# SciML/NeuralPDE.jl

Measured on NVIDIA H100. Metric: collocation-points/sec (loss+grad), higher is better.
Workload: dtype f32

## Files before the change

### neuralpde.jl_b200/csrc/tc_common.cuh

```cuda
#pragma once
#include <cuda_runtime.h>
#include <stdint.h>
#include "tc_types.h"
#include "ffma_kernel.cuh"
#include "tc_prims.cuh"
#include "tail.cuh"

namespace pinn {

constexpr int kNH = kTcThreads / 128;
static_assert(kTcThreads == 512, "the MMA chains are spread over four warpgroups");
constexpr int GW = 4;
constexpr int GWB = 2;

template <int N>
__device__ __forceinline__ float pick(const float* v, int idx) {
  float r = v[0];
#pragma unroll
  for (int i = 1; i < N; ++i) r = (idx == i) ? v[i] : r;
  return r;
}
template <int N>
__device__ __forceinline__ void add_at(float* v, int idx, float x) {
#pragma unroll
// ... 194 lines not shown
  int tl_max, off_P, off_misc, off_ones, mx_dim, mx_taps;
};
__device__ __forceinline__ void cta_base_init(CtaBase& cs, const TcCommonArgs& a, float* partial) {
  cs.partial = partial;
  cs.tl_max = a.tl_max; cs.off_P = a.off_P; cs.off_misc = a.off_misc; cs.off_ones = a.off_ones;
  cs.mx_dim = a.mx_dim; cs.mx_taps = a.mx_taps;
#ifdef PINN_DEBUG
  cs.dbg = (blockIdx.x == 0) ? a.dbg : nullptr;
#else
  cs.dbg = nullptr;
#endif
  cs.dbg_n = 0;
  dbg_mark(&cs, 1);
}

struct Misc {
  float *Xs, *taps, *tapbar, *scratch, *qws;
  double* tsum;
  uint64_t* bar_ld;
};
__device__ __forceinline__ Misc misc_of(uint8_t* m, int mx_dim, int mx_taps) {
  Misc r;
  r.Xs = reinterpret_cast<float*>(m);             m += mx_dim * kTcPts * 4;
  r.taps = reinterpret_cast<float*>(m);           m += mx_taps * kTcPts * 4;
  r.tapbar = reinterpret_cast<float*>(m);         m += mx_taps * kTcPts * 4;
  r.scratch = reinterpret_cast<float*>(m);        m += kTcMaxC * kTcPts * 4;
  r.qws = reinterpret_cast<float*>(m);            m += kTcPts * 4;
  r.tsum = reinterpret_cast<double*>(m);          m += PINN_MAX_TERMS * 8;
  r.bar_ld = reinterpret_cast<uint64_t*>(m);
  return r;
}

template <int N1, int N2>
struct PassInfo {
  int L, TL, d_in, n1w, nL;
  int dir1[N1 > 0 ? N1 : 1];
  Chan<N1, N2> ch;
};
template <int N1, int N2>
__device__ __forceinline__ void load_pass(PassInfo<N1, N2>& pi, const DevNet& net, const DevChan& dc) {
  pi.L = net.n_layers; pi.TL = pi.L - 2; pi.d_in = net.dims[0]; pi.n1w = net.dims[1]; pi.nL = net.dims[pi.L - 1];
#pragma unroll
  for (int j = 0; j < N1; ++j) pi.dir1[j] = dc.dir1[j];
#pragma unroll
  for (int s = 0; s < N2; ++s) { pi.ch.sa[s] = dc.s_a[s]; pi.ch.sb[s] = dc.s_b[s]; }
}

template <int W, int N1, int N2>
__device__ __forceinline__ void first_layer_elem(uint32_t fpa, const PassInfo<N1, N2>& pi, const float (&x)[PINN_MAX_IN],
                                                 int o, float* zz) {
  using F = FpBlock<W>;
  float s = lds_f32(fpa + (F::B1 + o) * 4);
  const uint32_t wa = fpa + (F::W1 + o * 8) * 4;
  if (pi.d_in <= 3) {
    s = fmaf(lds_f32(wa), x[0], s);
    if (pi.d_in >= 2) s = fmaf(lds_f32(wa + 4), x[1], s);
    if (pi.d_in == 3) s = fmaf(lds_f32(wa + 8), x[2], s);
  } else {
#pragma unroll
    for (int k = 0; k < PINN_MAX_IN; ++k)
      if (k < pi.d_in) s = fmaf(lds_f32(wa + k * 4), x[k], s);
  }
  zz[0] = s;
#pragma unroll
  for (int j = 0; j < N1; ++j) zz[1 + j] = lds_f32(fpa + (F::W1 + o * 8 + pi.dir1[j]) * 4);
#pragma unroll
  for (int j = 0; j < N2; ++j) zz[1 + N1 + j] = 0.f;
}

__device__ __forceinline__ void wait_bar(uint64_t* bar, uint32_t& phase) {
  tc::mbar_wait(bar, phase);
  phase ^= 1u;
}

static __device__ __noinline__ void mma_chain(uint32_t d, uint64_t adesc, uint64_t bdesc, uint32_t a_step, uint32_t b_step, int nk,
                                          uint32_t idesc, uint32_t acc_first) {
  const int n = (int)(idesc & 0xffu), ta = (int)((idesc >> 8) & 1u), tb = (int)((idesc >> 9) & 1u);
  const uint32_t dcol = d & 0xffffu, j = dcol >> 4;
  const uint32_t lbo = (uint32_t)((adesc >> 16) & 0x3fffu) << 4;
  const int wg = (int)(threadIdx.x >> 7);
#pragma unroll 1
  for (int h = 0; h < 2; ++h) {
    if (h == 1 && ta && lbo == 0) break;
    if (wg != 2 * (__popc(j) & 1) + h) continue;
    const uint64_t a = adesc + ((h ? (ta ? lbo : 8192u) : 0u) >> 4);
    if (ta == 0 && tb == 0) tc::wg_chain_n<0, 0>(n, dcol, h, a, bdesc, a_step, b_step, nk, acc_first);
    else if (ta == 0) tc::wg_chain_n<0, 1>(n, dcol, h, a, bdesc, a_step, b_step, nk, acc_first);
    else if (tb == 0) tc::wg_chain_n<1, 0>(n, dcol, h, a, bdesc, a_step, b_step, nk, acc_first);
    else tc::wg_chain_n<1, 1>(n, dcol, h, a, bdesc, a_step, b_step, nk, acc_first);
  }
}

struct Tid {
  int tid, warp, lane, q, hh, p;
  uint32_t lane_addr;
};
__device__ __forceinline__ Tid tid_of() {
  Tid t;
  t.tid = threadIdx.x; t.warp = t.tid >> 5; t.lane = t.tid & 31; t.q = t.warp & 3; t.hh = t.warp >> 2;
  t.p = t.q * 32 + t.lane;
  t.lane_addr = (uint32_t)(t.q * 32) << 16;
  return t;
}


__device__ __forceinline__ void cta_setup(const TcCommonArgs& a, const Misc& ms, float* partial, long long n_theta, bool want_grad) {
  extern __shared__ __align__(1024) uint8_t smem[];
  const int tid = threadIdx.x;
  if (want_grad) {
    const long long n4 = n_theta / 4;
    float4* p4 = reinterpret_cast<float4*>(partial);
    if ((reinterpret_cast<uintptr_t>(partial) & 15) == 0) {
      for (long long i = tid; i < n4; i += kTcThreads) p4[i] = make_float4(0.f, 0.f, 0.f, 0.f);
      for (long long i = n4 * 4 + tid; i < n_theta; i += kTcThreads) partial[i] = 0.f;
    } else {
      for (long long i = tid; i < n_theta; i += kTcThreads) partial[i] = 0.f;
    }
  }
  if (tid < PINN_MAX_TERMS) ms.tsum[tid] = 0.0;
  if (tid < 64) {
    const int r = tid >> 3, ch = tid & 7;
    *reinterpret_cast<uint4*>(smem + a.off_ones + r * 128 + ch * 16) = make_uint4(ch == r ? 0x00003f80u : 0u, 0u, 0u, 0u);
  }
}

template <int W>
__device__ __forceinline__ void stage_fp_block(float* fp, const DevNet& net, const float* theta) {
  using F = FpBlock<W>;
  const int tid = threadIdx.x, L = net.n_layers;
  for (int i = tid; i < F::SIZE; i += kTcThreads) fp[i] = 0.f;
  __syncthreads();
  const int n1w = net.dims[1], d_in = net.dims[0];
  const long long w0 = net.w_off[0], b0 = net.b_off[0];
  for (int i = tid; i < n1w * d_in; i += kTcThreads) {
    const int o = i % n1w, k = i / n1w;
    fp[F::W1 + o * 8 + k] = __ldg(&theta[w0 + i]);
  }
  for (int i = tid; i < n1w; i += kTcThreads) fp[F::B1 + i] = __ldg(&theta[b0 + i]);
  for (int i = tid; i < (L - 2) * W; i += kTcThreads) {
    const int l = 1 + i / W, o = i & (W - 1);
    if (o < net.dims[l + 1]) fp[F::BT + (l - 1) * W + o] = __ldg(&theta[net.b_off[l] + o]);
  }
  const int nL = net.dims[L - 1];
  const long long wl = net.w_off[L - 1], bl = net.b_off[L - 1];
  for (int i = tid; i < nL; i += kTcThreads) fp[F::WL + i] = __ldg(&theta[wl + i]);
  if (tid == 0) fp[F::BL] = __ldg(&theta[bl]);
}

struct TileRef {
  int ti;
  long long p0, n_pts;
};

__device__ __forceinline__ TileRef stage_tile(const TcCommonArgs& a, const DevProblem& P, const Misc& ms, int tile,
                                              uint32_t& ld_phase) {
  const int tid = threadIdx.x;
  int ti = 0;
  while (ti + 1 < P.n_terms && tile >= a.dyn[ti + 1].tile0) ++ti;
  const DevTerm& tm = P.terms[ti];
  const long long p0 = (long long)(tile - a.dyn[ti].tile0) * kTcPts;
  const long long n_pts = a.dyn[ti].n;
  const float* pts = reinterpret_cast<const float*>(a.dyn[ti].pts);
  const float* qw = reinterpret_cast<const float*>(a.dyn[ti].qw);
  if (tid < (int)((sizeof(DevTerm) + 127) / 128)) tc::prefetch_l1(reinterpret_cast<const char*>(&tm) + tid * 128);
  const int dim = tm.dim, n_taps = tm.n_taps, weighted = tm.weighted;
  const float* tile_src = pts + p0 * dim;
  const bool bulk_tile = (p0 + kTcPts <= n_pts) && dim <= kTcMaxC && ((reinterpret_cast<uintptr_t>(tile_src) & 15) == 0);
  if (bulk_tile) {
    if (tid == 0) {
      tc::mbar_arrive_expect_tx(ms.bar_ld, (uint32_t)(dim * kTcPts * 4));
      tc::bulk_load(ms.scratch, tile_src, (uint32_t)(dim * kTcPts * 4), ms.bar_ld);
    }
    wait_bar(ms.bar_ld, ld_phase);
    if (tid < kTcPts)
      for (int r = 0; r < dim; ++r) ms.Xs[r * kTcPts + tid] = ms.scratch[tid * dim + r];
  } else {
    for (int i = tid; i < dim * kTcPts; i += kTcThreads) {
      int pp = i / dim, r = i - pp * dim;
      long long gp = p0 + pp;
      if (gp >= n_pts) gp = n_pts - 1;
      ms.Xs[r * kTcPts + pp] = pts[gp * dim + r];
    }
  }
  if (tid < kTcPts) {
    long long gp = p0 + tid;
    float w = 0.f;
    if (gp < n_pts) w = weighted ? qw[gp] : 1.f;
    ms.qws[tid] = w;
  }
  for (int i = tid; i < n_taps * kTcPts; i += kTcThreads) ms.tapbar[i] = 0.f;
  __syncthreads();
  return TileRef{ti, p0, n_pts};
}

__device__ __forceinline__ void residual_step(const TcCommonArgs& a, const DevProblem& P, const DevTerm& tm, const Misc& ms,
                                              const TileRef& tr, uint8_t* region, size_t region_bytes, float* partial,
                                              bool want_grad) {
  const int tid = threadIdx.x, lane = tid & 31;
  const int n_instr = tm.n_instr, n_taps = tm.n_taps;
  DevInstr* sprog = reinterpret_cast<DevInstr*>(region);
  float* sval = reinterpret_cast<float*>(region + 8192);
  const bool prog_sm = (size_t)8192 + (size_t)2 * n_instr * kTcPts * 4 <= region_bytes;
  if (prog_sm) {
    const int nw = n_instr * (int)(sizeof(DevInstr) / 4);
    const int* src = reinterpret_cast<const int*>(tm.prog);
    for (int i = tid; i < nw; i += kTcThreads) reinterpret_cast<int*>(sprog)[i] = __ldg(src + i);
    __syncthreads();
  }
  if (tid < kTcPts) {
    float pbar[PINN_MAX_PARAMS];
#pragma unroll
    for (int j = 0; j < PINN_MAX_PARAMS; ++j) pbar[j] = 0.f;
    float r;
    if (prog_sm) {
      r = run_program_t<float, kTcPts, true>(sprog, n_instr, a.theta + P.param_off, ms.Xs, ms.taps, ms.tapbar, pbar, tid,
                                             want_grad, sval, sval + n_instr * kTcPts);
    } else {
      r = run_program<float, kTcPts>(tm, a.theta + P.param_off, ms.Xs, ms.taps, ms.tapbar, pbar, tid, want_grad);
    }
    const float w = ms.qws[tid];
    double s = (double)w * (double)r * (double)r;
#pragma unroll
    for (int o = 16; o > 0; o >>= 1) s += __shfl_xor_sync(0xffffffffu, s, o);
    if (lane == 0) atomicAdd(&ms.tsum[tr.ti], s);
    if (a.mode == 2) {
      long long gp = tr.p0 + tid;
      if (gp < tr.n_pts) a.resid_out[gp] = r;
    }
    if (want_grad) {
      const float g = (float)a.seed[tr.ti] * w * 2.f * r;
      for (int tt = 0; tt < n_taps; ++tt) ms.tapbar[tt * kTcPts + tid] *= g;
      const int n_params = P.n_params;
      for (int j = 0; j < n_params; ++j) {
        float v = warp_sum<float>(pbar[j] * g);
        if (lane == 0) atomicAdd(&partial[P.param_off + j], v);
      }
    }
  }
  __syncthreads();
}

struct DbgSpan {
  long long c0;
  unsigned long long g0;
};
__device__ __forceinline__ DbgSpan dbg_span_begin(const long long* dbg) {
  DbgSpan s{0, 0};
#ifdef PINN_DEBUG
  if (dbg && threadIdx.x == 0) {
    s.c0 = clock64();
    asm volatile("mov.u64 %0, %globaltimer;" : "=l"(s.g0));
  }
#endif
  return s;
}

template <typename CS>
__device__ __forceinline__ void cta_finish(const TcCommonArgs& a, const CS& cs, const DbgSpan& span, const Misc& ms,
                                           const DevProblem& P, bool want_grad) {
  extern __shared__ __align__(1024) uint8_t smem[];
  const int tid = threadIdx.x;
#ifdef PINN_DEBUG
  if (tid == 0 && cs.dbg) cs.dbg[999] = cs.dbg_n;
  if (a.dbg && tid == 0 && blockIdx.x < 250) {
    unsigned long long g1;
    unsigned int smid;
    asm volatile("mov.u64 %0, %globaltimer;" : "=l"(g1));
    asm volatile("mov.u32 %0, %smid;" : "=r"(smid));
    long long* rec = a.dbg + 1000 + 4 * blockIdx.x;
    rec[0] = (long long)span.g0; rec[1] = (long long)g1; rec[2] = clock64() - span.c0; rec[3] = smid;
  }
#endif
  if (tid < PINN_MAX_TERMS) a.term_sums[(long long)blockIdx.x * PINN_MAX_TERMS + tid] = ms.tsum[tid];
  if (a.tail.state)
    fused_tail<float, kTcThreads>(a.tail, a.partial, a.partial_stride, a.term_sums, P.n_theta, P.n_terms, want_grad ? 1 : 0,
                                  reinterpret_cast<float*>(smem + a.off_P));
}


template <int C, typename CS>
__device__ __forceinline__ void finish_forward(CS* cs, const DevTerm& tm, int slot, const Misc& ms, const float* bl, const Tid& t,
                                               const float (&u)[C]) {
  __syncthreads();
  dbg_mark(cs, 15);
#pragma unroll
  for (int c = 0; c < C; ++c) atomicAdd(&ms.scratch[c * kTcPts + t.p], u[c]);
  __syncthreads();
  if (t.hh == 0) {
    float s[C];
#pragma unroll
    for (int c = 0; c < C; ++c) s[c] = ms.scratch[c * kTcPts + t.p];
    s[0] += *bl;
    const int n_taps = tm.n_taps;
    for (int tt = 0; tt < n_taps; ++tt)
      if (tm.tap_slot[tt] == slot) {
        const int tch = tm.tap_ch[tt];
        float v = s[0];
#pragma unroll
        for (int c = 1; c < C; ++c) v = (tch == c) ? s[c] : v;
        ms.taps[tt * kTcPts + t.p] = v;
      }
  }
  __syncthreads();
  dbg_mark(cs, 16);
}

template <int C>
__device__ __forceinline__ void gather_ubar(const DevTerm& tm, int slot, const Misc& ms, int p, float (&ub)[C]) {
#pragma unroll
  for (int c = 0; c < C; ++c) ub[c] = 0.f;
  const int n_taps = tm.n_taps;
  for (int tt = 0; tt < n_taps; ++tt)
    if (tm.tap_slot[tt] == slot) {
      const float g = ms.tapbar[tt * kTcPts + p];
      const int tch = tm.tap_ch[tt];
#pragma unroll
      for (int c = 0; c < C; ++c) ub[c] += (tch == c) ? g : 0.f;
    }
}

template <int C>
__device__ __forceinline__ void last_layer_grad(const Tid& t, const float (&ub)[C], int nL, float* gw, float* gb, uint32_t u_tile,
// ... 149 lines not shown
```

### neuralpde.jl_b200/csrc/tc_kernel.cu

```cuda
#include "tc_common.cuh"

namespace pinn {

using Fp = FpBlock<kTcW>;

struct CtaShared : CtaBase {
  int split, off_Q;
  uint8_t* stash;
  TcNetSmem nets[PINN_MAX_NETS];
};

struct LoopCtx {
  uint32_t fp;
  uint32_t bt;
  uint32_t tP;
  uint32_t tQ;
  float* gb;
  float* gw;
  uint32_t taddr;
  int act, split, p, lane, g0, g1, flag;
  __device__ __forceinline__ LoopCtx(uint32_t fp_, uint32_t bt_, uint32_t tP_, uint32_t tQ_, const Tid& t, int act_, int ng,
                                     int flag_, int split_ = 0, float* gb_ = nullptr, float* gw_ = nullptr)
      : fp(fp_), bt(bt_), tP(tP_), tQ(tQ_), gb(gb_), gw(gw_), taddr(t.lane_addr), act(act_), split(split_), p(t.p), lane(t.lane),
        g0(t.hh * (ng / kNH)), g1((t.hh + 1) * (ng / kNH)), flag(flag_) {}
// ... 20 lines not shown
      for (int c = 0; c < C; ++c) zz[c] = mk2(za[c], zb2[c]);
      chain_fwd<N1, N2, PURE, AK, P2>(lc.act, pi.ch, zz, hv);
#pragma unroll
      for (int c = 0; c < C; ++c) { h[c][i] = hv[c].v.x; h[c][i + 1] = hv[c].v.y; }
      if (lc.flag) {
        const float w0 = lds_f32(lc.fp + (Fp::WL + g * GW + i) * 4), w1 = lds_f32(lc.fp + (Fp::WL + g * GW + i + 1) * 4);
#pragma unroll
        for (int c = 0; c < C; ++c) u[c] = fmaf(w1, hv[c].v.y, fmaf(w0, hv[c].v.x, u[c]));
      }
    }
#pragma unroll
    for (int c = 0; c < C; ++c) store_half(lc.tP + c * kTileBytes, lc.tQ + c * kTileBytes, lc.p, g * GW, h[c], lc.split != 0);
  }
#pragma unroll
  for (int c = 0; c < C; ++c) up[c] = u[c];
}

template <int C, int NK, bool SPLIT>
__device__ __forceinline__ void fwd_mma(float (&d)[C][16], uint32_t sP, uint32_t sQ, uint32_t whi, uint32_t wlo) {
  const int wg = threadIdx.x >> 7;
  const uint32_t aoff = (wg & 1) * 8192u, boff = (wg >> 1) * 32u * 128u;
  const uint64_t dwhi = tc::make_desc(whi + boff, 0, 1024), dwlo = tc::make_desc(wlo + boff, 0, 1024);
  tc::wgmma_fence();
#pragma unroll
  for (int c = 0; c < C; ++c) {
    const uint64_t dahi = tc::make_desc(sP + c * kTileBytes + aoff, 0, 1024);
    const uint64_t dalo = tc::make_desc(sQ + c * kTileBytes + aoff, 0, 1024);
#pragma unroll
    for (int pr = 0; pr < (SPLIT ? 3 : 1); ++pr) {
      const uint64_t a = (pr == 2) ? dalo : dahi, b = (pr == 1) ? dwlo : dwhi;
#pragma unroll
      for (int k = 0; k < NK; ++k)
        tc::wgmma_n32<0, 0>(d[c], a + 2 * k, b + 2 * k, (pr | k) ? 1u : 0u);
    }
  }
  tc::wgmma_commit();
  tc::wgmma_wait0();
}
template <int C>
__device__ __forceinline__ void fwd_mma_any(float (&d)[C][16], uint32_t sP, uint32_t sQ, uint32_t whi, uint32_t wlo, int nk,
                                            bool split) {
  switch (nk * 2 + (split ? 1 : 0)) {
    case 2: fwd_mma<C, 1, false>(d, sP, sQ, whi, wlo); break;
    case 3: fwd_mma<C, 1, true>(d, sP, sQ, whi, wlo); break;
    case 4: fwd_mma<C, 2, false>(d, sP, sQ, whi, wlo); break;
    case 5: fwd_mma<C, 2, true>(d, sP, sQ, whi, wlo); break;
    case 6: fwd_mma<C, 3, false>(d, sP, sQ, whi, wlo); break;
    case 7: fwd_mma<C, 3, true>(d, sP, sQ, whi, wlo); break;
    case 8: fwd_mma<C, 4, false>(d, sP, sQ, whi, wlo); break;
    default: fwd_mma<C, 4, true>(d, sP, sQ, whi, wlo); break;
  }
}

template <int N1, int N2, bool PURE, int AK, int C>
__device__ __forceinline__ void tl_fwd_frag(const float (&d)[C][16], const LoopCtx lc, const Chan<N1, N2> ch, float* scratch) {
  const int wg = threadIdx.x >> 7, w = (threadIdx.x >> 5) & 3;
  const int row0 = 64 * (wg & 1) + 16 * w + (lc.lane >> 2);
  const int col0 = 32 * (wg >> 1) + 2 * (lc.lane & 3);
  float u[2][C];
#pragma unroll
  for (int r = 0; r < 2; ++r)
#pragma unroll
    for (int c = 0; c < C; ++c) u[r][c] = 0.f;
#pragma unroll
  for (int i = 0; i < 16; i += 2) {
    const int rh = (i >> 1) & 1;
    const int row = row0 + 8 * rh, col = col0 + 8 * (i >> 2);
    P2 zz[C], hv[C];
    zz[0] = mk2(d[0][i] + lds_f32(lc.bt + col * 4), d[0][i + 1] + lds_f32(lc.bt + (col + 1) * 4));
#pragma unroll
    for (int c = 1; c < C; ++c) zz[c] = mk2(d[c][i], d[c][i + 1]);
    chain_fwd<N1, N2, PURE, AK, P2>(lc.act, ch, zz, hv);
    const uint32_t off = tc::swz_off(row, col);
#pragma unroll
    for (int c = 0; c < C; ++c) {
      const uint32_t hx = tc::pack_bf16(hv[c].v.x, hv[c].v.y);
      asm volatile("st.shared.b32 [%0], %1;" ::"r"(lc.tP + c * kTileBytes + off), "r"(hx) : "memory");
      if (lc.split)
        asm volatile("st.shared.b32 [%0], %1;" ::"r"(lc.tQ + c * kTileBytes + off), "r"(bf16x2_lo(hv[c].v.x, hv[c].v.y, hx))
                     : "memory");
    }
    if (lc.flag) {
      const float w0 = lds_f32(lc.fp + (Fp::WL + col) * 4), w1 = lds_f32(lc.fp + (Fp::WL + col + 1) * 4);
#pragma unroll
      for (int c = 0; c < C; ++c) u[rh][c] = fmaf(w1, hv[c].v.y, fmaf(w0, hv[c].v.x, u[rh][c]));
    }
  }
  if (lc.flag) {
#pragma unroll
    for (int r = 0; r < 2; ++r)
#pragma unroll
      for (int c = 0; c < C; ++c) {
        float s = u[r][c];
        s += __shfl_xor_sync(0xffffffffu, s, 1);
        s += __shfl_xor_sync(0xffffffffu, s, 2);
        if ((lc.lane & 3) == 0) atomicAdd(&scratch[c * kTcPts + row0 + 8 * r], s);
      }
  }
}

template <int C, int NKO>
__device__ __forceinline__ void dgrad_mma(float (&d)[C][16], uint32_t sP, uint32_t whi) {
  const uint32_t poff = (threadIdx.x >> 7) * 32u * 128u;
  const uint64_t dw = tc::make_desc(whi, 0, 1024);
  tc::wgmma_fence();
#pragma unroll
  for (int c = 0; c < C; ++c) {
    const uint64_t dz = tc::make_desc(sP + c * kTileBytes + poff, 0, 1024);
#pragma unroll
    for (int k = 0; k < NKO; ++k)
      tc::wgmma_n32<1, 0>(d[c], dw + 128 * k, dz + 2 * k, k ? 1u : 0u);
  }
  tc::wgmma_commit();
  tc::wgmma_wait0();
}
template <int C>
__device__ __forceinline__ void dgrad_mma_any(float (&d)[C][16], uint32_t sP, uint32_t whi, int nko) {
  switch (nko) {
    case 1: dgrad_mma<C, 1>(d, sP, whi); break;
    case 2: dgrad_mma<C, 2>(d, sP, whi); break;
    case 3: dgrad_mma<C, 3>(d, sP, whi); break;
    default: dgrad_mma<C, 4>(d, sP, whi); break;
  }
}
template <int C>
__device__ __forceinline__ void wgrad_mma(float (&dw)[32], float (&db)[8], uint32_t sP, uint32_t sQ, uint32_t s_ones) {
  const uint32_t poff = (threadIdx.x >> 7) * 32u * 128u;
  const uint64_t d1 = tc::make_desc(s_ones, 0, 0);
  tc::wgmma_fence();
#pragma unroll
  for (int c = 0; c < C; ++c) {
    const uint64_t dh = tc::make_desc(sQ + c * kTileBytes + poff, 0, 1024), dz = tc::make_desc(sP + c * kTileBytes + poff, 0, 1024);
#pragma unroll
    for (int k = 0; k < 2; ++k) tc::wgmma_n64<1, 1>(dw, dh + 128 * k, dz + 128 * k, (c | k) ? 1u : 0u);
  }
  const uint64_t dz0 = tc::make_desc(sP + poff, 0, 1024);
#pragma unroll
  for (int k = 0; k < 2; ++k) tc::wgmma_n16<1, 1>(db, dz0 + 128 * k, d1, k ? 1u : 0u);
  tc::wgmma_commit();
  tc::wgmma_wait0();
}

template <int NF>
__device__ __forceinline__ void frag_store_rows(float* base, int ld, const float (&d)[NF]) {
  const int w = (threadIdx.x >> 5) & 3, lane = threadIdx.x & 31;
  const bool odd = (lane & 1) != 0;
  float* row = base + (16 * w + (lane >> 2) + (odd ? 8 : 0)) * ld + 4 * ((lane >> 1) & 1);
#pragma unroll
  for (int j = 0; j < NF / 4; ++j) {
    const float r0 = __shfl_xor_sync(0xffffffffu, odd ? d[4 * j] : d[4 * j + 2], 1);
    const float r1 = __shfl_xor_sync(0xffffffffu, odd ? d[4 * j + 1] : d[4 * j + 3], 1);
    *reinterpret_cast<float4*>(row + 8 * j) =
        odd ? make_float4(r0, r1, d[4 * j + 2], d[4 * j + 3]) : make_float4(d[4 * j], d[4 * j + 1], r0, r1);
  }
}

template <int N1, int N2, bool PURE, int AK, int C>
__device__ __forceinline__ void tl_bwd_frag(const float (&d)[C][16], const LoopCtx lc, const Chan<N1, N2> ch, const float* ubs) {
  const int wg = threadIdx.x >> 7, w = (threadIdx.x >> 5) & 3;
  const int row0 = 64 * (wg & 1) + 16 * w + (lc.lane >> 2);
  const int col0 = 32 * (wg >> 1) + 2 * (lc.lane & 3);
  const float* hbar = tc::s_acc + TM_X * kAccRows;
#pragma unroll
  for (int i = 0; i < 16; i += 2) {
    const int row = row0 + 8 * ((i >> 1) & 1), col = col0 + 8 * (i >> 2);
    P2 zz[C], hv[C], zv[C];
    zz[0] = mk2(d[0][i] + lds_f32(lc.bt + col * 4), d[0][i + 1] + lds_f32(lc.bt + (col + 1) * 4));
#pragma unroll
    for (int c = 1; c < C; ++c) zz[c] = mk2(d[c][i], d[c][i + 1]);
    if (lc.flag) {
      const float w0 = lds_f32(lc.fp + (Fp::WL + col) * 4), w1 = lds_f32(lc.fp + (Fp::WL + col + 1) * 4);
#pragma unroll
      for (int c = 0; c < C; ++c) {
        const float u = ubs[c * kTcPts + row];
        hv[c] = mk2(w0 * u, w1 * u);
      }
    } else {
#pragma unroll
      for (int c = 0; c < C; ++c) hv[c] = mk2(hbar[(c * 64 + col) * kAccRows + row], hbar[(c * 64 + col + 1) * kAccRows + row]);
    }
    chain_bwd<N1, N2, PURE, AK, P2>(lc.act, ch, zz, hv, zv);
    const uint32_t off = tc::swz_off(row, col);
#pragma unroll
    for (int c = 0; c < C; ++c)
      asm volatile("st.shared.b32 [%0], %1;" ::"r"(lc.tP + c * kTileBytes + off), "r"(tc::pack_bf16(zv[c].v.x, zv[c].v.y))
                   : "memory");
  }
}

template <int N1, int N2, bool PURE, int AK>
__device__ __forceinline__ void l0_bwd_store_loop(const LoopCtx lc, const PassInfo<N1, N2> pi, const float* xp) {
  constexpr int C = 1 + N1 + N2;
  float x[PINN_MAX_IN];
#pragma unroll
  for (int k = 0; k < PINN_MAX_IN; ++k) x[k] = xp[k];
#pragma unroll 1
  for (int g = lc.g0; g < lc.g1; ++g) {
    float hb[C][GWB];
#pragma unroll
    for (int c = 0; c < C; ++c) acc_ldg(lc.taddr + TM_X + c * 64 + g * GWB, hb[c]);
#pragma unroll
    for (int i = 0; i < GWB; i += 2) {
      float za[C], zb2[C];
      first_layer_elem<kTcW>(lc.fp, pi, x, g * GWB + i, za);
      first_layer_elem<kTcW>(lc.fp, pi, x, g * GWB + i + 1, zb2);
      P2 zz[C], hv[C], zv[C];
#pragma unroll
      for (int c = 0; c < C; ++c) { zz[c] = mk2(za[c], zb2[c]); hv[c] = mk2(hb[c][i], hb[c][i + 1]); }
      chain_bwd<N1, N2, PURE, AK, P2>(lc.act, pi.ch, zz, hv, zv);
#pragma unroll
      for (int c = 0; c <= N1; ++c) { hb[c][i] = zv[c].v.x; hb[c][i + 1] = zv[c].v.y; }
    }
#pragma unroll
    for (int c = 0; c <= N1; ++c) store_half(lc.tP + c * kTileBytes, lc.tP, lc.p, g * GWB, hb[c], false);
  }
}

template <int N1, int N2, bool PURE, int AK>
__device__ __forceinline__ void l0_bwd_loop(const LoopCtx lc, const PassInfo<N1, N2> pi, const float* xp, const float* ubp) {
  constexpr int C = 1 + N1 + N2;
  float x[PINN_MAX_IN], ub[C];
#pragma unroll
  for (int k = 0; k < PINN_MAX_IN; ++k) x[k] = xp[k];
#pragma unroll
  for (int c = 0; c < C; ++c) ub[c] = ubp[c];
  const int re = reduceg_elem(lc.lane);
  const bool rlead = reduceg_lead(lc.lane);
  const int n1w = pi.n1w;
#pragma unroll 1
  for (int g = lc.g0; g < lc.g1; ++g) {
    float hb[C][GW];
    if (!lc.flag) {
#pragma unroll
      for (int c = 0; c < C; ++c) acc_ldg(lc.taddr + TM_X + c * 64 + g * GW, hb[c]);
    } else {
#pragma unroll
      for (int i = 0; i < GW; ++i) {
        const float wl = lds_f32(lc.fp + (Fp::WL + g * GW + i) * 4);
#pragma unroll
        for (int c = 0; c < C; ++c) hb[c][i] = wl * ub[c];
      }
    }
    float zv0[GW], zvd[N1 > 0 ? N1 : 1][GW];
#pragma unroll
    for (int i = 0; i < GW; ++i) {
      float zz[C], hv[C], zv[C];
      first_layer_elem<kTcW>(lc.fp, pi, x, g * GW + i, zz);
#pragma unroll
      for (int c = 0; c < C; ++c) hv[c] = hb[c][i];
      chain_bwd<N1, N2, PURE, AK, float>(lc.act, pi.ch, zz, hv, zv);
      zv0[i] = zv[0];
#pragma unroll
      for (int jd = 0; jd < N1; ++jd) zvd[jd][i] = zv[1 + jd];
    }
    const float bs = warp_reduceg(zv0, lc.lane);
    if (rlead) atomicAdd(lc.gb + g * GW + re, bs);
#pragma unroll
    for (int k = 0; k < PINN_MAX_IN; ++k) {
      if (k < pi.d_in) {
        float gk[GW];
#pragma unroll
        for (int i = 0; i < GW; ++i) {
          float gg = zv0[i] * x[k];
#pragma unroll
          for (int jd = 0; jd < N1; ++jd) gg += (pi.dir1[jd] == k) ? zvd[jd][i] : 0.f;
          gk[i] = gg;
        }
        const float gs = warp_reduceg(gk, lc.lane);
        if (rlead) atomicAdd(lc.gw + g * GW + re + (long long)n1w * k, gs);
      }
    }
  }
}

template <int N1, int N2, bool PURE, int AK>
__device__ __noinline__ uint32_t net_forward(CtaShared* cs, const DevProblem* Pp, const DevTerm* tmp, int slot,
                                             int want_grad, uint32_t phase) {
  extern __shared__ __align__(1024) uint8_t smem[];
  constexpr int C = 1 + N1 + N2;
  const DevTerm& tm = *tmp;
  const int net_id = tm.used_net[slot];
  const DevNet& net = Pp->nets[net_id];
  const DevChan& dc = tm.chan[slot];
  const TcNetSmem ns = cs->nets[net_id];
  const float* fp = reinterpret_cast<const float*>(smem + ns.fp);
  uint8_t* tP = smem + cs->off_P;
  uint8_t* tQ = smem + cs->off_Q;
  const Misc ms = misc_of(smem + cs->off_misc, cs->mx_dim, cs->mx_taps);
  const uint32_t accm = 0;
  const bool split = cs->split != 0;
  PassInfo<N1, N2> pi;
  load_pass<N1, N2>(pi, net, dc);
  const int TL = pi.TL;
  const Tid t = tid_of();
  const int tid = t.tid, p = t.p;
  float x[PINN_MAX_IN];
#pragma unroll
  for (int k = 0; k < PINN_MAX_IN; ++k) x[k] = (k < pi.d_in) ? ms.Xs[dc.rows[k] * kTcPts + p] : 0.f;
  uint8_t* stash_slot = cs->stash + (size_t)slot * cs->tl_max * kTcMaxC * kTileBytes;

  dbg_mark(cs, 10);
  float u[C];
#pragma unroll
  for (int c = 0; c < C; ++c) u[c] = 0.f;
  if (tid < C * kTcPts / 4) reinterpret_cast<float4*>(ms.scratch)[tid] = make_float4(0.f, 0.f, 0.f, 0.f);
  {
    const LoopCtx lc(tc::smem_u32(fp), tc::smem_u32(fp), tc::smem_u32(tP), tc::smem_u32(tQ), t, net.acts[0], pi.n1w / GW, TL == 0, split);
    l0_fwd_loop<N1, N2, PURE, AK>(lc, pi, x, u);
  }
  for (int l = 1; l <= TL; ++l) {
    const int n_in = net.dims[l], n_out = net.dims[l + 1];
    const int act = net.acts[l];
    tc::fence_async_smem();
    __syncthreads();
    dbg_mark(cs, 11);
    if (want_grad && tid == 0) {
      for (int c = 0; c < C; ++c)
        tc::bulk_store(stash_slot + (size_t)(l - 1) * kTcMaxC * kTileBytes + (size_t)c * kTileBytes, tP + c * kTileBytes, kTileBytes);
      tc::bulk_commit();
    }
    float d[C][16];
    {
      const uint32_t sP = tc::smem_u32(tP), sQ = tc::smem_u32(tQ);
      const uint32_t whi = tc::smem_u32(smem + ns.w_hi[l - 1]), wlo = tc::smem_u32(smem + ns.w_lo[l - 1]);
      const int nk = n_in / 16;
      fwd_mma_any<C>(d, sP, sQ, whi, wlo, nk, split);
    }
    dbg_mark(cs, 13);
    if (want_grad && tid == 0) tc::bulk_wait_read0();
    __syncthreads();
    dbg_mark(cs, 14);
    const LoopCtx lc(tc::smem_u32(fp), tc::smem_u32(fp) + (Fp::BT + (l - 1) * 64) * 4, tc::smem_u32(tP), tc::smem_u32(tQ), t, act, 0, l == TL, split);
    tl_fwd_frag<N1, N2, PURE, AK, C>(d, lc, pi.ch, ms.scratch);
  }
  finish_forward<C>(cs, tm, slot, ms, fp + Fp::BL, t, u);
  return phase;
}

template <int N1, int N2, bool PURE, int AK>
__device__ __noinline__ uint32_t net_backward(CtaShared* cs, const DevProblem* Pp, const DevTerm* tmp, int slot,
                                              uint32_t phase) {
  extern __shared__ __align__(1024) uint8_t smem[];
  constexpr int C = 1 + N1 + N2;
  const DevTerm& tm = *tmp;
  const int net_id = tm.used_net[slot];
  const DevNet& net = Pp->nets[net_id];
  const DevChan& dc = tm.chan[slot];
  const TcNetSmem ns = cs->nets[net_id];
  const float* fp = reinterpret_cast<const float*>(smem + ns.fp);
  uint8_t* tP = smem + cs->off_P;
  uint8_t* tQ = smem + cs->off_Q;
  const Misc ms = misc_of(smem + cs->off_misc, cs->mx_dim, cs->mx_taps);
  const uint32_t accm = 0;
  float* partial = cs->partial;
  PassInfo<N1, N2> pi;
  load_pass<N1, N2>(pi, net, dc);
  const int L = pi.L, TL = pi.TL;
  const Tid t = tid_of();
  const int tid = t.tid, p = t.p;
  uint32_t ld_phase = (phase >> 1) & 1u;
  float x[PINN_MAX_IN];
#pragma unroll
  for (int k = 0; k < PINN_MAX_IN; ++k) x[k] = (k < pi.d_in) ? ms.Xs[dc.rows[k] * kTcPts + p] : 0.f;
  uint8_t* stash_slot = cs->stash + (size_t)slot * cs->tl_max * kTcMaxC * kTileBytes;

  dbg_mark(cs, 20);
  float ub[C];
  gather_ubar<C>(tm, slot, ms, p, ub);
  if (t.hh == 0) {
#pragma unroll
    for (int c = 0; c < C; ++c) ms.scratch[c * kTcPts + p] = ub[c];
  }
  last_layer_grad<C>(t, ub, pi.nL, partial + net.w_off[L - 1], partial + net.b_off[L - 1], tc::smem_u32(tQ), tc::smem_u32(tP),
                     kTileBytes, 0u, accm + TM_Y, kTcW);

  const uint32_t sP = tc::smem_u32(tP), sQ = tc::smem_u32(tQ);
  const int wg = tid >> 7;
  float* hand = tc::s_acc + TM_X * kAccRows;
  float* wpart = reinterpret_cast<float*>(tP);
  float* bpart = ms.scratch;
  static_assert(4 * 64 <= kTcMaxC * kTcPts, "the bias partials fit ms.scratch");
  for (int l = TL; l >= 1; --l) {
    const int n_in = net.dims[l], n_out = net.dims[l + 1];
    const int act = net.acts[l];
    float* gb = partial + net.b_off[l];
    float* gw = partial + net.w_off[l];
    const float* bt = fp + Fp::BT + (l - 1) * 64;
    const uint32_t whi = tc::smem_u32(smem + ns.w_hi[l - 1]);
    dbg_mark(cs, 21);
    if (tid == 0 && l == TL) {
      const uint8_t* src = stash_slot + (size_t)(l - 1) * kTcMaxC * kTileBytes;
      tc::mbar_arrive_expect_tx(ms.bar_ld, C * kTileBytes);
      for (int c = 0; c < C; ++c) tc::bulk_load(tQ + c * kTileBytes, src + (size_t)c * kTileBytes, kTileBytes, ms.bar_ld);
    }
    wait_bar(ms.bar_ld, ld_phase);
    dbg_mark(cs, 22);
    {
      float d[C][16];
      fwd_mma_any<C>(d, sQ, sQ, whi, whi, n_in / 16, false);
      __syncthreads();
      dbg_mark(cs, 24);
      const LoopCtx lc(tc::smem_u32(fp), tc::smem_u32(bt), sP, sQ, t, act, 0, l == TL);
      tl_bwd_frag<N1, N2, PURE, AK, C>(d, lc, pi.ch, ms.scratch);
    }
    tc::fence_async_smem();
    __syncthreads();
    dbg_mark(cs, 26);
    {
      float d[C][16];
      dgrad_mma_any<C>(d, sP, whi, n_out / 16);
#pragma unroll
      for (int c = 0; c < C; ++c) frag_store_rows(hand + c * 64 * kAccRows + 32 * wg, kAccRows, d[c]);
    }
    dbg_mark(cs, 27);
    {
      float dw[32], db[8];
      wgrad_mma<C>(dw, db, sP, sQ, tc::smem_u32(smem + cs->off_ones));
      __syncthreads();
      if (tid == 0 && l > 1) {
        const uint8_t* src = stash_slot + (size_t)(l - 2) * kTcMaxC * kTileBytes;
        tc::mbar_arrive_expect_tx(ms.bar_ld, C * kTileBytes);
        for (int c = 0; c < C; ++c) tc::bulk_load(tQ + c * kTileBytes, src + (size_t)c * kTileBytes, kTileBytes, ms.bar_ld);
      }
      frag_store_rows(wpart + wg * 64 * 64, 64, dw);
      if ((t.lane & 3) == 0) {
        const int o = 16 * (t.warp & 3) + (t.lane >> 2);
        bpart[wg * 64 + o] = db[0];
        bpart[wg * 64 + o + 8] = db[2];
      }
    }
    __syncthreads();
    dbg_mark(cs, 28);
#pragma unroll 1
    for (int e = tid; e < 64 * 64; e += kTcThreads) {
      const int k = e >> 6, o = e & 63;
      if (k < n_in && o < n_out) atomicAdd(gw + o + (long long)n_out * k, ((wpart[e] + wpart[4096 + e]) + wpart[8192 + e]) + wpart[12288 + e]);
    }
    if (tid < n_out) atomicAdd(gb + tid, ((bpart[tid] + bpart[64 + tid]) + bpart[128 + tid]) + bpart[192 + tid]);
  }

  {
    __syncthreads();
    dbg_mark(cs, 29);
    const int act0 = net.acts[0];
    float* gb0 = partial + net.b_off[0];
    float* gw0 = partial + net.w_off[0];
    if (TL == 0) {
      const LoopCtx lc(tc::smem_u32(fp), tc::smem_u32(fp), sP, sQ, t, act0, pi.n1w / GW, 1, 0, gb0, gw0);
      l0_bwd_loop<N1, N2, PURE, AK>(lc, pi, x, ub);
    } else {
      coord_tiles<N1>(t, sQ, x, pi.dir1, N2 > 0);
      const LoopCtx lc(tc::smem_u32(fp), tc::smem_u32(fp), sP, sQ, t, act0, pi.n1w / GWB, 0);
      l0_bwd_store_loop<N1, N2, PURE, AK>(lc, pi, x);
      layer0_grad<N1>(t, sP, kTileBytes, 0u, sQ, N2 > 0, accm + TM_Y, kTcW, pi.n1w, pi.d_in, gw0, gb0);
    }
  }
  __syncthreads();
  dbg_mark(cs, 30);
  return (ld_phase << 1) | (phase & 1u);
}


__global__ void __launch_bounds__(kTcThreads, 1) tc_loss_grad_kernel(const __grid_constant__ TcArgs args) {
  extern __shared__ __align__(1024) uint8_t smem[];
  __shared__ CtaShared cs;
  const int tid = threadIdx.x;
  const DevProblem* Pp = args.prob;
  const DevProblem& P = *Pp;
  const Misc ms = misc_of(smem + args.off_misc, args.mx_dim, args.mx_taps);
  float* partial = args.partial + (long long)blockIdx.x * args.partial_stride;
  const bool want_grad = (args.mode == 0);
  const float* theta = args.theta;
  const DbgSpan span = dbg_span_begin(args.dbg);

  for (long long i = (long long)tid * 32; i < args.n_theta; i += (long long)kTcThreads * 32) tc::prefetch_l2(theta + i);
  {
    const char* nets0 = reinterpret_cast<const char*>(&Pp->nets[0]);
    const char* terms0 = reinterpret_cast<const char*>(&Pp->terms[0]);
    const int nb_nets = args.n_nets * (int)sizeof(DevNet), nb_terms = args.n_terms * (int)sizeof(DevTerm);
    if (tid == 0) tc::prefetch_l2(Pp);
    for (int o = tid * 128; o < nb_nets; o += kTcThreads * 128) tc::prefetch_l2(nets0 + o);
    for (int o = tid * 128; o < nb_terms; o += kTcThreads * 128) tc::prefetch_l2(terms0 + o);
    const int tile = args.tile_begin + (int)blockIdx.x;
    if (tile < args.tile_end && tid < 32) {
      int ti = 0;
      while (ti + 1 < args.n_terms && tile >= args.dyn[ti + 1].tile0) ++ti;
      const long long p0 = (long long)(tile - args.dyn[ti].tile0) * kTcPts;
      const long long row_bytes = 4ll * args.term_dim[ti];
      const long long off = p0 * row_bytes + (long long)tid * 128;
      if (off < args.dyn[ti].n * row_bytes) tc::prefetch_l2(reinterpret_cast<const char*>(args.dyn[ti].pts) + off);
    }
  }
  if (tid == 0) {
    tc::mbar_init(ms.bar_ld, 1);
    tc::fence_barrier_init();
    cs.split = args.split; cs.off_Q = args.off_Q;
    cs.stash = args.stash + (long long)blockIdx.x * args.stash_per_cta;
    for (int k = 0; k < PINN_MAX_NETS; ++k) cs.nets[k] = args.nets[k];
    cta_base_init(cs, args, partial);
  }
  if (tid == 0) tc::s_acc = args.acc + (size_t)blockIdx.x * kAccCols * kAccRows;
  cta_setup(args, ms, partial, P.n_theta, want_grad);
  for (int kn = 0; kn < P.n_nets; ++kn) {
    const DevNet& net = P.nets[kn];
    const TcNetSmem& ns = args.nets[kn];
    if (ns.fp < 0) continue;
    stage_fp_block<kTcW>(reinterpret_cast<float*>(smem + ns.fp), net, theta);
    const int L = net.n_layers;
    {
      constexpr int kItMax = kTcMaxTL * 512 / kTcThreads;
      const int n_items = (L - 2) * 512;
      float w[kItMax][8];
#pragma unroll
      for (int it = 0; it < kItMax; ++it) {
        const int i = tid + it * kTcThreads;
        if (i < n_items) {
          const int l = 1 + i / 512, r = i & 511;
          const int o = r & 63, kc = r >> 6;
          const int n_in = net.dims[l], n_out = net.dims[l + 1];
          const long long woff = net.w_off[l];
#pragma unroll
          for (int e = 0; e < 8; ++e) {
            const int k = kc * 8 + e;
            w[it][e] = (o < n_out && k < n_in) ? __ldg(&theta[woff + o + (long long)n_out * k]) : 0.f;
          }
        }
      }
#pragma unroll
      for (int it = 0; it < kItMax; ++it) {
        const int i = tid + it * kTcThreads;
        if (i < n_items) {
          const int l = 1 + i / 512, r = i & 511;
          const int o = r & 63, kc = r >> 6;
          uint8_t* thi = smem + ns.w_hi[l - 1];
          uint8_t* tlo = smem + ns.w_lo[l - 1];
          const float* v = w[it];
          uint32_t h[4];
#pragma unroll
          for (int e = 0; e < 4; ++e) h[e] = tc::pack_bf16(v[2 * e], v[2 * e + 1]);
          *reinterpret_cast<uint4*>(thi + tc::swz_chunk(o, kc)) = make_uint4(h[0], h[1], h[2], h[3]);
          if (args.split)
            *reinterpret_cast<uint4*>(tlo + tc::swz_chunk(o, kc)) = make_uint4(
                bf16x2_lo(v[0], v[1], h[0]), bf16x2_lo(v[2], v[3], h[1]), bf16x2_lo(v[4], v[5], h[2]), bf16x2_lo(v[6], v[7], h[3]));
        }
      }
    }
  }
  tc::fence_async_smem();
  __syncthreads();
  dbg_mark(&cs, 2);
  uint32_t phase = 0;

  for (int tile = args.tile_begin + blockIdx.x; tile < args.tile_end; tile += gridDim.x) {
    if (tid >= 128 && tid < 128 + (int)((sizeof(DevNet) * PINN_MAX_NETS + 127) / 128))
      tc::prefetch_l1(reinterpret_cast<const char*>(&P.nets[0]) + (tid - 128) * 128);
    uint32_t ldp = (phase >> 1) & 1u;
    const TileRef tr = stage_tile(args, P, ms, tile, ldp);
    phase = (phase & 1u) | (ldp << 1);
    const DevTerm* tmp = &P.terms[tr.ti];
    const DevTerm& tm = *tmp;
    const int n_used = tm.n_used;
    dbg_mark(&cs, 3);

    for (int slot = 0; slot < n_used; ++slot) {
      const int k1 = tm.chan[slot].n1, k2 = tm.chan[slot].n2, pu = tm.chan[slot].pure;
      const int ak = args.net_ak[tm.used_net[slot]];
      PINN_TC_DISPATCH(kTcMaxC, k1, k2, pu, ak, (phase = net_forward<A1, A2, PU, AK>(&cs, Pp, tmp, slot, want_grad ? 1 : 0, phase)));
    }

    dbg_mark(&cs, 4);
    residual_step(args, P, tm, ms, tr, smem + args.off_Q, (size_t)args.off_Q_bytes, partial, want_grad);

    dbg_mark(&cs, 5);
    if (want_grad) {
      if (tid == 0) tc::bulk_wait0();
      __syncthreads();
      dbg_mark(&cs, 6);
      for (int slot = n_used - 1; slot >= 0; --slot) {
        const int k1 = tm.chan[slot].n1, k2 = tm.chan[slot].n2, pu = tm.chan[slot].pure;
        const int ak = args.net_ak[tm.used_net[slot]];
        if (n_used > 1) {
          PINN_TC_DISPATCH(kTcMaxC, k1, k2, pu, ak, (phase = net_forward<A1, A2, PU, AK>(&cs, Pp, tmp, slot, 0, phase)));
        }
        PINN_TC_DISPATCH(kTcMaxC, k1, k2, pu, ak, (phase = net_backward<A1, A2, PU, AK>(&cs, Pp, tmp, slot, phase)));
      }
    }
  }

  __syncthreads();
  dbg_mark(&cs, 7);
  cta_finish(args, cs, span, ms, P, want_grad);
}

size_t tc_misc_bytes(int mx_dim, int mx_taps) {
  return (size_t)mx_dim * kTcPts * 4 + 2 * (size_t)mx_taps * kTcPts * 4 + (size_t)kTcMaxC * kTcPts * 4 + kTcPts * 4 +
         PINN_MAX_TERMS * 8 + 16 + 16;
}

cudaError_t tc_launch(const TcArgs& a, int grid, size_t smem, cudaStream_t st) {
  return launch_fused_kernel<tc_loss_grad_kernel>(a, grid, kTcThreads, smem, st);
}

}
```

Baseline: 94.02 million.

## Compute last-layer and layer-0 grads in registers, drop atomics, prefetch first tile

Several changes land together. The last-layer and layer-0 weight gradients are now computed with wgmma into register fragments and reduced through shared memory, replacing the previous accumulator-based path. Per-CTA gradient partials are written directly, with a first-write flag per net, instead of through atomicAdd, and a vectorised float4 path handles 64-wide layers. The first tile's bulk load is also issued during CTA setup to overlap it with weight staging. The main risks are correctness of the fresh flag if a CTA gets no tiles for a net, and that non-atomic writes assume partials are private to each CTA.

Result: faster. 96.60 million (median of 6 runs) (+2.7%).

```diff
diff --git a/neuralpde.jl_b200/csrc/tc_common.cuh b/neuralpde.jl_b200/csrc/tc_common.cuh
--- a/neuralpde.jl_b200/csrc/tc_common.cuh
+++ b/neuralpde.jl_b200/csrc/tc_common.cuh
@@ -370,8 +370,9 @@
   long long p0, n_pts;
 };
 
+template <bool PRE = false>
 __device__ __forceinline__ TileRef stage_tile(const TcCommonArgs& a, const DevProblem& P, const Misc& ms, int tile,
-                                              uint32_t& ld_phase) {
+                                              uint32_t& ld_phase, bool issued = false) {
   const int tid = threadIdx.x;
   int ti = 0;
   while (ti + 1 < P.n_terms && tile >= a.dyn[ti + 1].tile0) ++ti;
@@ -385,7 +386,7 @@
   const float* tile_src = pts + p0 * dim;
   const bool bulk_tile = (p0 + kTcPts <= n_pts) && dim <= kTcMaxC && ((reinterpret_cast<uintptr_t>(tile_src) & 15) == 0);
   if (bulk_tile) {
-    if (tid == 0) {
+    if (tid == 0 && !(PRE && issued)) {
       tc::mbar_arrive_expect_tx(ms.bar_ld, (uint32_t)(dim * kTcPts * 4));
       tc::bulk_load(ms.scratch, tile_src, (uint32_t)(dim * kTcPts * 4), ms.bar_ld);
     }
diff --git a/neuralpde.jl_b200/csrc/tc_kernel.cu b/neuralpde.jl_b200/csrc/tc_kernel.cu
--- a/neuralpde.jl_b200/csrc/tc_kernel.cu
+++ b/neuralpde.jl_b200/csrc/tc_kernel.cu
@@ -196,6 +196,111 @@
     const float r1 = __shfl_xor_sync(0xffffffffu, odd ? d[4 * j + 1] : d[4 * j + 3], 1);
     *reinterpret_cast<float4*>(row + 8 * j) =
         odd ? make_float4(r0, r1, d[4 * j + 2], d[4 * j + 3]) : make_float4(d[4 * j], d[4 * j + 1], r0, r1);
+  }
+}
+
+__device__ __forceinline__ void partial_add(float* g, float v, bool fresh) {
+  if (fresh) *g = v + 0.f;
+  else *g += v;
+}
+
+template <int C>
+__device__ __forceinline__ void last_layer_grad_regs(const Tid& t, const float (&ub)[C], int nL, float* gw, float* gb, uint32_t sU,
+                                                     uint32_t sH, float* part, bool fresh) {
+  float bsum = 0.f;
+  if (t.hh == 0) {
+    bsum = warp_sum<float>(ub[0]);
+#pragma unroll
+    for (int c = 0; c < C; ++c) {
+      const uint32_t hi = tc::pack_bf16(ub[c], 0.f);
+      const uint32_t v = hi | (bf16x2_lo(ub[c], 0.f, hi) << 16);
+      uint32_t w[8];
+#pragma unroll
+      for (int i = 0; i < 8; ++i) w[i] = (i == c) ? v : 0u;
+      sts_v4(sU + c * kTileBytes + tc::swz_chunk(t.p, 0), w[0], w[1], w[2], w[3]);
+      sts_v4(sU + c * kTileBytes + tc::swz_chunk(t.p, 1), w[4], w[5], w[6], w[7]);
+    }
+  }
+  tc::fence_async_smem();
+  __syncthreads();
+  const int wg = t.tid >> 7;
+  float d[8];
+  {
+    const uint32_t poff = wg * 32u * 128u;
+    tc::wgmma_fence();
+#pragma unroll
+    for (int c = 0; c < C; ++c) {
+      const uint64_t dh = tc::make_desc(sH + c * kTileBytes + poff, 0, 1024), du = tc::make_desc(sU + c * kTileBytes + poff, 0, 1024);
+#pragma unroll
+      for (int k = 0; k < 2; ++k) tc::wgmma_n16<1, 1>(d, dh + 128 * k, du + 128 * k, (c | k) ? 1u : 0u);
+    }
+    tc::wgmma_commit();
+    tc::wgmma_wait0();
+  }
+  __syncthreads();
+  const int o0 = 16 * (t.warp & 3) + (t.lane >> 2);
+#pragma unroll
+  for (int c = 0; c < C; ++c) {
+    const int j = 4 * (c >> 2);
+    if ((t.lane & 3) == (c & 3)) {
+      part[(wg * C + c) * 64 + o0] = d[j] + d[j + 1];
+      part[(wg * C + c) * 64 + o0 + 8] = d[j + 2] + d[j + 3];
+    }
+  }
+  if (t.hh == 0 && t.lane == 0) part[4 * C * 64 + t.q] = bsum;
+  __syncthreads();
+  if (t.tid < nL) {
+    const int o = t.tid;
+    float acc = 0.f;
+#pragma unroll
+    for (int c = 0; c < C; ++c)
+      acc += ((part[c * 64 + o] + part[(C + c) * 64 + o]) + part[(2 * C + c) * 64 + o]) + part[(3 * C + c) * 64 + o];
+    partial_add(gw + o, acc, fresh);
+  }
+  if (t.tid == kTcThreads - 1) {
+    const float* bp = part + 4 * C * 64;
+    partial_add(gb, ((bp[0] + bp[1]) + bp[2]) + bp[3], fresh);
+  }
+}
+
+template <int N1, bool XLO>
+__device__ __forceinline__ void layer0_grad_regs(const Tid& t, uint32_t sZ, uint32_t sB, int n1w, int d_in, float* gw0, float* gb0,
+                                                 float* part, bool fresh) {
+  tc::fence_async_smem();
+  __syncthreads();
+  const int wg = t.tid >> 7;
+  float d[8];
+  {
+    const uint32_t poff = wg * 32u * 128u;
+    const uint64_t dz0 = tc::make_desc(sZ + poff, 0, 1024), dx = tc::make_desc(sB + poff, 0, 1024);
+    tc::wgmma_fence();
+#pragma unroll
+    for (int k = 0; k < 2; ++k) tc::wgmma_n16<1, 1>(d, dz0 + 128 * k, dx + 128 * k, k ? 1u : 0u);
+    if (XLO) {
+      const uint64_t dlo = tc::make_desc(sB + (1 + N1) * kTileBytes + poff, 0, 1024);
+#pragma unroll
+      for (int k = 0; k < 2; ++k) tc::wgmma_n16<1, 1>(d, dz0 + 128 * k, dlo + 128 * k, 1u);
+    }
+#pragma unroll
+    for (int j = 0; j < N1; ++j) {
+      const uint64_t dz = tc::make_desc(sZ + (1 + j) * kTileBytes + poff, 0, 1024);
+      const uint64_t de = tc::make_desc(sB + (1 + j) * kTileBytes + poff, 0, 1024);
+#pragma unroll
+      for (int k = 0; k < 2; ++k) tc::wgmma_n16<1, 1>(d, dz + 128 * k, de + 128 * k, 1u);
+    }
+    tc::wgmma_commit();
+    tc::wgmma_wait0();
+  }
+  __syncthreads();
+  frag_store_rows(part + wg * 64 * 16, 16, d);
+  __syncthreads();
+#pragma unroll
+  for (int it = 0; it < 64 * 16 / kTcThreads; ++it) {
+    const int e = t.tid + it * kTcThreads, o = e >> 4, n = e & 15;
+    if (o < n1w && (n < d_in || n == 8)) {
+      float* g = (n == 8) ? gb0 + o : gw0 + o + (long long)n1w * n;
+      partial_add(g, ((part[e] + part[1024 + e]) + part[2048 + e]) + part[3072 + e], fresh);
+    }
   }
 }
 
@@ -383,7 +488,7 @@
 
 template <int N1, int N2, bool PURE, int AK>
 __device__ __noinline__ uint32_t net_backward(CtaShared* cs, const DevProblem* Pp, const DevTerm* tmp, int slot,
-                                              uint32_t phase) {
+                                              uint32_t phase, bool fresh) {
   extern __shared__ __align__(1024) uint8_t smem[];
   constexpr int C = 1 + N1 + N2;
   const DevTerm& tm = *tmp;
@@ -395,7 +500,6 @@
   uint8_t* tP = smem + cs->off_P;
   uint8_t* tQ = smem + cs->off_Q;
   const Misc ms = misc_of(smem + cs->off_misc, cs->mx_dim, cs->mx_taps);
-  const uint32_t accm = 0;
   float* partial = cs->partial;
   PassInfo<N1, N2> pi;
   load_pass<N1, N2>(pi, net, dc);
@@ -415,8 +519,8 @@
 #pragma unroll
     for (int c = 0; c < C; ++c) ms.scratch[c * kTcPts + p] = ub[c];
   }
-  last_layer_grad<C>(t, ub, pi.nL, partial + net.w_off[L - 1], partial + net.b_off[L - 1], tc::smem_u32(tQ), tc::smem_u32(tP),
-                     kTileBytes, 0u, accm + TM_Y, kTcW);
+  last_layer_grad_regs<C>(t, ub, pi.nL, partial + net.w_off[L - 1], partial + net.b_off[L - 1], tc::smem_u32(tQ), tc::smem_u32(tP),
+                          reinterpret_cast<float*>(tP), fresh);
 
   const uint32_t sP = tc::smem_u32(tP), sQ = tc::smem_u32(tQ);
   const int wg = tid >> 7;
@@ -475,12 +579,37 @@
     }
     __syncthreads();
     dbg_mark(cs, 28);
+    if (n_out == 64 && (reinterpret_cast<uintptr_t>(gw) & 15) == 0) {
+      const int e = 8 * tid;
+      if ((e >> 6) < n_in) {
+        float4* g = reinterpret_cast<float4*>(gw + e);
+        const float4* w4 = reinterpret_cast<const float4*>(wpart + e);
+        float4 v[2];
+        if (fresh) {
+          v[0] = v[1] = make_float4(0.f, 0.f, 0.f, 0.f);
+        } else {
+          v[0] = g[0];
+          v[1] = g[1];
+        }
+#pragma unroll
+        for (int h = 0; h < 2; ++h) {
+          const float4 a = w4[h], b = w4[1024 + h], c = w4[2048 + h], d = w4[3072 + h];
+          v[h].x += ((a.x + b.x) + c.x) + d.x;
+          v[h].y += ((a.y + b.y) + c.y) + d.y;
+          v[h].z += ((a.z + b.z) + c.z) + d.z;
+          v[h].w += ((a.w + b.w) + c.w) + d.w;
+          g[h] = v[h];
+        }
+      }
+    } else {
 #pragma unroll 1
-    for (int e = tid; e < 64 * 64; e += kTcThreads) {
-      const int k = e >> 6, o = e & 63;
-      if (k < n_in && o < n_out) atomicAdd(gw + o + (long long)n_out * k, ((wpart[e] + wpart[4096 + e]) + wpart[8192 + e]) + wpart[12288 + e]);
-    }
-    if (tid < n_out) atomicAdd(gb + tid, ((bpart[tid] + bpart[64 + tid]) + bpart[128 + tid]) + bpart[192 + tid]);
+      for (int e = tid; e < 64 * 64; e += kTcThreads) {
+        const int k = e >> 6, o = e & 63;
+        if (k < n_in && o < n_out)
+          partial_add(gw + o + (long long)n_out * k, ((wpart[e] + wpart[4096 + e]) + wpart[8192 + e]) + wpart[12288 + e], fresh);
+      }
+    }
+    if (tid < n_out) partial_add(gb + tid, ((bpart[tid] + bpart[64 + tid]) + bpart[128 + tid]) + bpart[192 + tid], fresh);
   }
 
   {
@@ -496,7 +625,7 @@
       coord_tiles<N1>(t, sQ, x, pi.dir1, N2 > 0);
       const LoopCtx lc(tc::smem_u32(fp), tc::smem_u32(fp), sP, sQ, t, act0, pi.n1w / GWB, 0);
       l0_bwd_store_loop<N1, N2, PURE, AK>(lc, pi, x);
-      layer0_grad<N1>(t, sP, kTileBytes, 0u, sQ, N2 > 0, accm + TM_Y, kTcW, pi.n1w, pi.d_in, gw0, gb0);
+      layer0_grad_regs<N1, (N2 > 0)>(t, sP, sQ, pi.n1w, pi.d_in, gw0, gb0, reinterpret_cast<float*>(tP), fresh);
     }
   }
   __syncthreads();
@@ -504,6 +633,19 @@
   return (ld_phase << 1) | (phase & 1u);
 }
 
+
+__device__ __forceinline__ void issue_tile_load(const TcArgs& a, const Misc& ms, int tile) {
+  if (tile >= a.tile_end) return;
+  int ti = 0;
+  while (ti + 1 < a.n_terms && tile >= a.dyn[ti + 1].tile0) ++ti;
+  const int dim = a.term_dim[ti];
+  const long long p0 = (long long)(tile - a.dyn[ti].tile0) * kTcPts;
+  const float* tile_src = reinterpret_cast<const float*>(a.dyn[ti].pts) + p0 * dim;
+  if ((p0 + kTcPts <= a.dyn[ti].n) && dim <= kTcMaxC && ((reinterpret_cast<uintptr_t>(tile_src) & 15) == 0)) {
+    tc::mbar_arrive_expect_tx(ms.bar_ld, (uint32_t)(dim * kTcPts * 4));
+    tc::bulk_load(ms.scratch, tile_src, (uint32_t)(dim * kTcPts * 4), ms.bar_ld);
+  }
+}
 
 __global__ void __launch_bounds__(kTcThreads, 1) tc_loss_grad_kernel(const __grid_constant__ TcArgs args) {
   extern __shared__ __align__(1024) uint8_t smem[];
@@ -535,9 +677,11 @@
       if (off < args.dyn[ti].n * row_bytes) tc::prefetch_l2(reinterpret_cast<const char*>(args.dyn[ti].pts) + off);
     }
   }
+  const int tile0 = args.tile_begin + (int)blockIdx.x;
   if (tid == 0) {
     tc::mbar_init(ms.bar_ld, 1);
     tc::fence_barrier_init();
+    issue_tile_load(args, ms, tile0);
     cs.split = args.split; cs.off_Q = args.off_Q;
     cs.stash = args.stash + (long long)blockIdx.x * args.stash_per_cta;
     for (int k = 0; k < PINN_MAX_NETS; ++k) cs.nets[k] = args.nets[k];
@@ -594,12 +738,13 @@
   __syncthreads();
   dbg_mark(&cs, 2);
   uint32_t phase = 0;
+  uint32_t fresh = (1u << PINN_MAX_NETS) - 1u;
 
   for (int tile = args.tile_begin + blockIdx.x; tile < args.tile_end; tile += gridDim.x) {
     if (tid >= 128 && tid < 128 + (int)((sizeof(DevNet) * PINN_MAX_NETS + 127) / 128))
       tc::prefetch_l1(reinterpret_cast<const char*>(&P.nets[0]) + (tid - 128) * 128);
     uint32_t ldp = (phase >> 1) & 1u;
-    const TileRef tr = stage_tile(args, P, ms, tile, ldp);
+    const TileRef tr = stage_tile<true>(args, P, ms, tile, ldp, tile == tile0);
     phase = (phase & 1u) | (ldp << 1);
     const DevTerm* tmp = &P.terms[tr.ti];
     const DevTerm& tm = *tmp;
@@ -626,7 +771,10 @@
         if (n_used > 1) {
           PINN_TC_DISPATCH(kTcMaxC, k1, k2, pu, ak, (phase = net_forward<A1, A2, PU, AK>(&cs, Pp, tmp, slot, 0, phase)));
         }
-        PINN_TC_DISPATCH(kTcMaxC, k1, k2, pu, ak, (phase = net_backward<A1, A2, PU, AK>(&cs, Pp, tmp, slot, phase)));
+        const int nid = tm.used_net[slot];
+        PINN_TC_DISPATCH(kTcMaxC, k1, k2, pu, ak,
+                         (phase = net_backward<A1, A2, PU, AK>(&cs, Pp, tmp, slot, phase, ((fresh >> nid) & 1u) != 0)));
+        fresh &= ~(1u << nid);
       }
     }
   }
```
